# adaly/gridnext

Hardware: AMD Instinct MI355X
Metric: spots/sec training throughput (multimodal f+g) (higher is better)
Workload: dtype f32; 1 GPU; C4: multimodal f(DenseNet-121 @128px + count-MLP 2000 genes) + hex g on 78x64 Visium grids, 1 array (4992 spots) per GPU per step, f frozen/eval (tutorial mode), g trained with Adam, masked CE; spots_per_array=4992, parallelism=dp1

## Files before the change

### gridnext_amd/_lib.py

```python
import ctypes
import os

import torch

_HERE = os.path.dirname(os.path.abspath(__file__))
LIB_PATH = os.environ.get('GNX_LIB') or os.path.join(_HERE, 'libgridnext_hip.so')

_P, _I, _L, _F, _D = ctypes.c_void_p, ctypes.c_int, ctypes.c_long, ctypes.c_float, ctypes.c_double
_LL = ctypes.c_longlong

SIGNATURES = {
    'gnx_hexconv_fwd': (_I, [_P, _P, _P, _P, _P, _I, _I, _I, _I, _I, _I, _P]),
    'gnx_hexconv_bwd_data': (_I, [_P, _P, _P, _P, _I, _I, _I, _I, _I, _I, _P]),
    'gnx_hexconv_bwd_weight_workspace': (_L, [_I, _I, _I, _I, _I]),
    'gnx_hexconv_bwd_weight': (_I, [_P, _P, _P, _P, _P, _P, _I, _I, _I, _I, _I, _I, _I, _P]),
    'gnx_hexconv_bwd_weight_batch': (_I, [_P, _I, _P]),
    'gnx_hexconv_k_fwd': (_I, [_P, _P, _P, _P, _I, _I, _I, _I, _I, _I, _I, _P]),
    'gnx_hexconv_k_bwd_data': (_I, [_P, _P, _P, _I, _I, _I, _I, _I, _I, _I, _P]),
    'gnx_hexconv_k_bwd_weight_workspace': (_L, [_I, _I, _I, _I, _I, _I]),
    'gnx_hexconv_k_bwd_weight': (_I, [_P, _P, _P, _P, _P, _I, _I, _I, _I, _I, _I, _I, _I, _P]),
    'gnx_gridconv_fwd': (_I, [_P, _P, _P, _P, _I, _I, _I, _I, _I, _I, _I, _P]),
    'gnx_gridconv_bwd_data': (_I, [_P, _P, _P, _I, _I, _I, _I, _I, _I, _I, _P]),
    'gnx_gridconv_bwd_weight_workspace': (_L, [_I, _I, _I, _I, _I, _I, _I]),
    'gnx_gridconv_bwd_weight': (_I, [_P, _P, _P, _P, _P, _I, _I, _I, _I, _I, _I, _I, _I, _P]),
# ... 79 lines not shown
    'gnx_trans_bwd_f16': (_I, [_P, _L, _P, _L, _P, _L, _L, _I, _I, _P, _P, _P, _P, _P, _P, _P, _P, _I, _P, _P]),
    'gnx_h16_cols_to_f32': (_I, [_P, _L, _P, _L, _L, _I, _P, _P, _P]),
    'gnx_stem_bwd_f16_workspace': (_L, [_L, _I]),
    'gnx_stem_bwd_f16': (_I, [_P, _P, _P, _P, _P, _P, _P, _L, _P, _P, _P, _P, _L, _I, _I, _P, _I, _P, _P]),
    'gnx_dense_layer_f16_pack': (_I, [_P, _P, _P, _P, _I, _P]),
    'gnx_dense_layer_f16': (_I, [_P, _L, _L, _I, _I, _P, _P, _P, _P, _P, _P, _P]),
    'gnx_dense_layer_f16_tape': (_I, [_P, _L, _L, _I, _I, _P, _P, _P, _P, _P, _P, _P, _L, _P]),
    'gnx_dense_bwd_f16_pack': (_I, [_P, _P, _P, _P, _I, _P]),
    'gnx_wgrad3x3_f16_lb': (_I, [_P, _L, _P, _L, _L, _P, _P, _L, _I, _P, _I, _P, _P]),
    'gnx_conv3x3_dgrad_bnrelu_bwd_f16_lb': (_I, [_P, _L, _P, _P, _L, _L, _P, _L, _I, _P, _P, _P, _P, _P, _P, _P, _I, _P, _P]),
    'gnx_conv3x3_bwd_f16_workspace': (_L, [_L]),
    'gnx_conv3x3_bwd_f16_lb': (_I, [_P, _L, _P, _P, _L, _L, _P, _P, _L, _I, _P, _P, _P, _P, _P, _P, _P, _I, _P, _P]),
    'gnx_conv1x1_dgrad_wgrad_bnrelu_bwd_f16_lb': (_I, [_P, _P, _P, _L, _L, _P, _L, _L, _L, _I, _P, _P, _P, _P, _P, _P, _P, _P, _P, _I,
                                                       _P, _P]),
    'gnx_tail_bwd_f16_lb': (_I, [_P, _L, _P, _L, _L, _P, _L, _L, _L, _I, _I, _P, _P, _P, _P, _P, _P, _P, _P, _I, _P, _P]),
    'gnx_trans_bwd_f16_lb': (_I, [_P, _L, _L, _P, _L, _L, _P, _L, _L, _L, _I, _I, _P, _P, _P, _P, _P, _P, _P, _P, _I, _P, _P]),
    'gnx_conv_stem_bnrelu_maxpool_f16mul_cb': (_I, [_P, _I, _P, _P, _L, _L, _I, _I, _I, _I, _I, _I, _I, _I, _P, _P, _P, _P]),
    'gnx_conv1x1_bnrelu_h16_cb': (_I, [_P, _L, _P, _P, _L, _L, _I, _I, _P, _P, _P, _P, _P]),
    'gnx_bnrelu_avgpool2_h16_cb': (_I, [_P, _L, _P, _L, _L, _I, _I, _P, _P, _P]),
    'gnx_transition_f16_pack': (_I, [_P, _P, _I, _I, _P]),
    'gnx_transition_f16': (_I, [_P, _L, _L, _I, _I, _I, _P, _P, _P, _P, _L, _P]),
    'gnx_transition_f16_tape': (_I, [_P, _L, _L, _I, _I, _I, _P, _P, _P, _P, _L, _P, _L, _P]),
    'gnx_bnrelu_avgpool_h16_cb': (_I, [_P, _L, _P, _L, _L, _I, _I, _P, _P, _P]),
    'gnx_conv3x3_bnrelu': (_I, [_P, _L, _P, _P, _L, _L, _I, _I, _I, _P, _P, _P]),
    'gnx_winograd_conv3x3_weights': (_I, [_P, _P, _I, _I, _P]),
    'gnx_conv3x3_winograd': (_I, [_P, _L, _P, _P, _L, _L, _I, _I, _I, _P]),
    'gnx_conv3x3_winograd_wide': (_I, [_P, _L, _P, _P, _L, _L, _I, _I, _I, _P]),
    'gnx_conv3x3_form': (_I, [_P, _L, _P, _P, _L, _L, _I, _I, _I, _P, _P, _P]),
    'gnx_conv3x3_winograd_form': (_I, [_P, _L, _P, _P, _L, _L, _I, _I, _I, _P]),
    'gnx_conv3x3_dgrad_bnrelu_bwd_form': (_I, [_P, _L, _P, _P, _L, _P, _L, _L, _I, _I, _I, _P, _P, _P, _P, _P, _P]),
    'gnx_conv3x3_f16_dma_form': (_I, [_P, _L, _P, _P, _L, _L, _I, _I, _I, _P]),
    'gnx_conv_stem': (_I, [_P, _P, _P, _L, _L, _I, _I, _I, _I, _I, _I, _I, _I, _P]),
    'gnx_conv_stem_bnrelu_maxpool': (_I, [_P, _P, _P, _L, _L, _I, _I, _I, _I, _I, _I, _I, _I, _P, _P, _P]),
    'gnx_conv_stem_bnrelu_maxpool_argmax': (_I, [_P, _P, _P, _L, _P, _L, _I, _I, _I, _I, _I, _I, _I, _I, _P, _P, _P]),
    'gnx_bnrelu_maxpool': (_I, [_P, _L, _P, _L, _L, _I, _I, _I, _P, _P, _P]),
    'gnx_bnrelu_avgpool': (_I, [_P, _L, _P, _L, _L, _I, _I, _P, _P, _P]),
    'gnx_spot_compact': (_I, [_P, _L, _L, _P, _P, _P, _P, _P]),
    'gnx_spot_broadcast_rows': (_I, [_P, _L, _L, _I, _P, _L, _P]),
    'gnx_conv_stem_bnrelu_maxpool_idx': (_I, [_P, _P, _P, _L, _L, _I, _I, _I, _I, _I, _I, _I, _I, _P, _P, _P, _L, _P]),
    'gnx_conv_stem_bnrelu_maxpool_u8_idx': (_I, [_P, _P, _P, _L, _L, _I, _I, _I, _I, _I, _I, _I, _I, _P, _P, _P, _P, _L, _P]),
    'gnx_bnrelu_avgpool_idx': (_I, [_P, _L, _P, _L, _L, _I, _I, _P, _P, _P, _L, _P]),
    'gnx_wgrad_workspace': (_L, [_L, _I, _I, _I]),
    'gnx_wgrad_bnrelu': (_I, [_P, _L, _P, _L, _P, _P, _P, _P, _L, _I, _I, _I, _I, _I, _I, _P]),
    'gnx_wgrad_bnrelu_batch': (_I, [_P, _I, _I, _P]),
    'gnx_transpose_weight': (_I, [_P, _P, _I, _I, _P]),
    'gnx_relayout_weights_batch': (_I, [_P, _I, _I, _P]),
    'gnx_repack_conv3x3_bwd': (_I, [_P, _P, _I, _I, _P]),
    'gnx_rows_broadcast': (_I, [_P, _L, _P, _L, _L, _I, _I, _F, _P]),
    'gnx_avgpool2_bwd': (_I, [_P, _L, _P, _L, _L, _I, _I, _P]),
    'gnx_maxpool_bwd': (_I, [_P, _L, _P, _L, _P, _L, _P, _L, _L, _I, _I, _I, _P, _P, _P]),
    'gnx_bnrelu_maxpool_argmax': (_I, [_P, _L, _P, _L, _P, _L, _I, _I, _I, _P, _P, _P]),
    'gnx_maxpool_bwd_argmax': (_I, [_P, _P, _L, _P, _L, _L, _I, _I, _I, _P]),
    'gnx_maxpool_bwd_argmax_bnrelu': (_I, [_P, _P, _L, _P, _L, _P, _P, _L, _L, _I, _I, _I, _P]),
    'gnx_conv0_wgrad_workspace': (_L, [_L, _I, _I, _I, _I, _I, _I, _I]),
    'gnx_conv0_wgrad': (_I, [_P, _P, _L, _P, _P, _L, _I, _I, _I, _I, _I, _I, _I, _I, _P]),
    'gnx_conv0_dgrad': (_I, [_P, _L, _P, _P, _L, _I, _I, _I, _I, _I, _I, _I, _P]),
    'gnx_softmax_rows': (_I, [_P, _L, _L, _I, _P, _L, _P, _P]),
    'gnx_gemm_f32': (_I, [_P, _L, _I, _P, _L, _I, _P, _P, _L, _L, _L, _L, _I, _P]),
    'gnx_gemm_f32_workspace': (_L, [_L, _L, _L]),
    'gnx_gemm_f32_ws': (_I, [_P, _L, _I, _P, _L, _I, _P, _P, _L, _L, _L, _L, _I, _P, _P]),
    'gnx_fingerprint128_split_bytes': (_L, []),
    'gnx_fingerprint128_batch_workspace': (_L, [ctypes.c_size_t, _I]),
    'gnx_fingerprint128_batch': (_I, [_P, ctypes.c_size_t, _I, _P, _P, _P]),
    'gnx_rgb_hist_u8_workspace': (_L, [ctypes.c_size_t]),
    'gnx_rgb_hist_u8': (_I, [_P, ctypes.c_size_t, _P, _P, _P]),
    'gnx_rgb_lut_u8': (_I, [_P, _P, ctypes.c_size_t, _P, _P]),
# ... 69 lines not shown
```

### gridnext_amd/csrc/stem_pool.hip

```cpp
#include <type_traits>
#include "fwd_common.h"

namespace {

__global__ __launch_bounds__(256) void u8_to_f32_kernel(const uint8_t* __restrict__ x8, float* __restrict__ out, long n4,
                                                        long hw4, int C, const float* __restrict__ nrm) {
    const long stride = (long)gridDim.x * blockDim.x;
    for (long i = (long)blockIdx.x * blockDim.x + threadIdx.x; i < n4; i += stride) {
        const int c = (int)((i / hw4) % C);
        const bool norm = nrm != nullptr && c < 3;
        const float mean = norm ? nrm[c] : 0.f, sd = norm ? nrm[3 + c] : 1.f, rsd = norm ? nrm[6 + c] : 1.f;
        const uint32_t wv = reinterpret_cast<const uint32_t*>(x8)[i];
        reinterpret_cast<float4*>(out)[i] = u8x4_pixels(wv, norm, mean, sd, rsd);
    }
}

constexpr int ST_BM = 128, ST_BN = 64;

__global__ __launch_bounds__(256) void conv_stem_kernel(const float* __restrict__ x, const float* __restrict__ w,
                                                        float* __restrict__ out, long ldc, long M, int Cin, int H,
                                                        int Wd, int Ho, int Wo, int O, int KH, int KW, int stride,
                                                        int pad) {
    extern __shared__ __attribute__((aligned(16))) float lds[];
    const int KC = KH * 8, LD = KC + 4;
// ... 131 lines not shown
            float4 na = a, nb0 = b0, nb1 = b1;
            if (step + 1 < NSTEP) {
                na = load_a(step + 1);
                nb0 = ld4(pb + (step + 1) * 8);
                nb1 = ld4(pb + 32 * LDB + (step + 1) * 8);
            }
            acc0 = __builtin_amdgcn_mfma_f32_32x32x2f32(a.x, b0.x, acc0, 0, 0, 0);
            acc1 = __builtin_amdgcn_mfma_f32_32x32x2f32(a.x, b1.x, acc1, 0, 0, 0);
            acc0 = __builtin_amdgcn_mfma_f32_32x32x2f32(a.y, b0.y, acc0, 0, 0, 0);
            acc1 = __builtin_amdgcn_mfma_f32_32x32x2f32(a.y, b1.y, acc1, 0, 0, 0);
            acc0 = __builtin_amdgcn_mfma_f32_32x32x2f32(a.z, b0.z, acc0, 0, 0, 0);
            acc1 = __builtin_amdgcn_mfma_f32_32x32x2f32(a.z, b1.z, acc1, 0, 0, 0);
            acc0 = __builtin_amdgcn_mfma_f32_32x32x2f32(a.w, b0.w, acc0, 0, 0, 0);
            acc1 = __builtin_amdgcn_mfma_f32_32x32x2f32(a.w, b1.w, acc1, 0, 0, 0);
            a = na; b0 = nb0; b1 = nb1;
            __builtin_amdgcn_sched_group_barrier(0x100, STRIDE % 2 == 0 ? 4 : 6, 0);
            __builtin_amdgcn_sched_group_barrier(0x008, 8, 0);
        }
#pragma unroll
        for (int r = 0; r < 16; ++r) {
            const int rr = 32 * wave + (r & 3) + 8 * (r >> 2) + 4 * h;
            const int oy = oy0 + (rr >> 4), ox = ox0 + (rr & 15);
            if (oy < Ho && ox < Wo) {
                float* o = out + ((img * Ho + oy) * (long)Wo + ox) * ldc;
                if (i < O) o[i] = acc0[r];
                if (32 + i < O) o[32 + i] = acc1[r];
            }
        }
    }
}

constexpr int SP_LDT = 40;
constexpr int SP_LDTH = 72;
template <int WO, bool H16 = false, bool U8 = false, bool IDX = false>
__global__ __launch_bounds__(256) void conv_stem_pool_kernel(const void* __restrict__ xv, const float* __restrict__ w,
                                                             float* __restrict__ out, long ldo, int H, int Wd, int O,
                                                             const float* __restrict__ scale,
                                                             const float* __restrict__ shift, long imgs,
                                                             const float* __restrict__ nrm,
                                                             unsigned char* __restrict__ amax = nullptr,
                                                             const int* __restrict__ src_idx = nullptr, long src_imgs = 0) {
    const float* __restrict__ x = reinterpret_cast<const float*>(xv);
    const uint8_t* __restrict__ x8 = reinterpret_cast<const uint8_t*>(xv);
    constexpr int CIN = 3, KH = 7, KW = 7, STRIDE = 2, PAD = 3;
    constexpr int RT = 128 / WO;
    constexpr int PH = STRIDE * (RT - 1) + KH, PW = ((WO - 1) * STRIDE + 8 + 1 + 1) & ~1;
    constexpr int F4R = WO * STRIDE / 4;
    constexpr int NPC = CIN * PH * F4R, NPRE = (NPC + 255) / 256;
    constexpr int NIT = (WO / 2) * 8 / 256;
    constexpr int KT = CIN * KH * 8, LDB = KT + 4;
    extern __shared__ __attribute__((aligned(16))) float lds[];
    auto store4 = [](float* o, long off, const float4& v) {
        if constexpr (H16) {
            typedef _Float16 half4 __attribute__((ext_vector_type(4)));
            const half4 hv = {(_Float16)v.x, (_Float16)v.y, (_Float16)v.z, (_Float16)v.w};
            *reinterpret_cast<half4*>(reinterpret_cast<_Float16*>(o) + off) = hv;
        } else {
            *reinterpret_cast<float4*>(o + off) = v;
        }
    };
    float* Bs = lds;
    float* Ps = lds + 64 * LDB;
    float* Ts = Ps + CIN * PH * PW;
    const int t = threadIdx.x, lane = t & 63, wave = t >> 6, h = lane >> 5, i = lane & 31;
    for (int idx = t; idx < 64 * KT; idx += 256) {
        const int n = idx / KT, rem = idx - n * KT;
        const int kx = rem & 7, cky = rem >> 3;
        float v = 0.f;
        if (n < O && kx < KW) v = w[((long)n * CIN * KH + cky) * KW + kx];
        Bs[n * LDB + rem] = v;
    }
    for (int idx = t; idx < CIN * PH * PW; idx += 256) Ps[idx] = 0.f;
    const int trow = 32 * wave + i;
    const float* pa = Ps + (STRIDE * (trow / WO)) * PW + STRIDE * (trow % WO) + 4 * h;
    const float* pb = Bs + i * LDB + 4 * h;
    const float sc0 = i < O ? scale[i] : 0.f, sh0 = i < O ? shift[i] : 0.f;
    const float sc1 = 32 + i < O ? scale[32 + i] : 0.f, sh1 = 32 + i < O ? shift[32 + i] : 0.f;
    const int c4 = t & 7, pxa = t >> 3;
    const int Ho2 = (H + 2 * PAD - KH) / STRIDE + 1;
    const int ntt = Ho2 / RT;

    float4 pre[U8 ? 1 : NPRE];
    uint32_t pre8[U8 ? NPRE : 1];
    bool in8[U8 ? NPRE : 1];
    auto fetch_patch = [&](long img, int tt) {
        const int iy0 = RT * tt * STRIDE - PAD;
#pragma unroll
        for (int q = 0; q < NPRE; ++q) {
            const int j = t + 256 * q;
            const int f4 = j % F4R, py = (j / F4R) % PH, c = (j / F4R) / PH;
            const int iy = iy0 + py;
            const bool inside = j < NPC && iy >= 0 && iy < H;
            if constexpr (U8) {
                pre8[q] = 0u;
                in8[q] = inside;
                if (inside)
                    pre8[q] = *reinterpret_cast<const uint32_t*>(x8 + ((img * CIN + c) * H + iy) * (long)Wd + 4 * f4);
            } else {
                pre[q] = make_float4(0.f, 0.f, 0.f, 0.f);
                if (inside) pre[q] = ld4(x + ((img * CIN + c) * H + iy) * (long)Wd + 4 * f4);
            }
        }
    };
    auto stash_patch = [&]() {
#pragma unroll
        for (int q = 0; q < NPRE; ++q) {
            const int j = t + 256 * q;
            if (j < NPC) {
                float* d = Ps + (j / F4R) * PW + PAD + 4 * (j % F4R);
                if constexpr (U8) {
                    const int c = (j / F4R) / PH;
                    const bool norm = nrm != nullptr;
                    const float4 v = in8[q] ? u8x4_pixels(pre8[q], norm, norm ? nrm[c] : 0.f, norm ? nrm[3 + c] : 1.f,
                                                          norm ? nrm[6 + c] : 1.f)
                                            : make_float4(0.f, 0.f, 0.f, 0.f);
                    d[0] = v.x; d[1] = v.y; d[2] = v.z; d[3] = v.w;
                } else {
                    d[0] = pre[q].x; d[1] = pre[q].y; d[2] = pre[q].z; d[3] = pre[q].w;
                }
            }
        }
    };
    auto src_of = [&](long img) -> long {
        if (src_idx == nullptr) return img;
        const long s = src_idx[img];
        return s < 0 ? 0 : (s < src_imgs ? s : src_imgs - 1);
    };
    __syncthreads();
    fetch_patch(src_of(blockIdx.x), 0);

    for (long img = blockIdx.x; img < imgs; img += gridDim.x) {
        const long src = src_of(img);
        float4 carry[2][NIT], carry2[2][NIT];
        unsigned cidx[2][NIT], cidx2[2][NIT];
        const float c0v = IDX ? -1.f : 0.f;
#pragma unroll
        for (int q = 0; q < NIT; ++q) {
            carry[0][q] = carry[1][q] = carry2[0][q] = carry2[1][q] = make_float4(c0v, c0v, c0v, c0v);
            cidx[0][q] = cidx[1][q] = cidx2[0][q] = cidx2[1][q] = 0u;
        }
        for (int tt = 0; tt < ntt; ++tt) {
            __syncthreads();
            stash_patch();
            {
                long nsrc = src;
                int nt2 = tt + 1;
                if (nt2 == ntt) {
                    nt2 = 0;
                    long nimg = img + gridDim.x;
                    if (nimg >= imgs) nimg = blockIdx.x;
                    nsrc = src_of(nimg);
                }
                fetch_patch(nsrc, nt2);
            }
            asm volatile("" ::: "memory");
            __syncthreads();
            f32x16 acc0, acc1;
#pragma unroll
            for (int r = 0; r < 16; ++r) { acc0[r] = 0.f; acc1[r] = 0.f; }
            auto load_a = [&](int step) {
                const float* ap = pa + ((step / KH) * PH + (step % KH)) * PW;
                const float2 lo = *reinterpret_cast<const float2*>(ap);
                const float2 hi = *reinterpret_cast<const float2*>(ap + 2);
                return make_float4(lo.x, lo.y, hi.x, hi.y);
            };
            constexpr int NSTEP = CIN * KH;
            float4 a = load_a(0), b0 = ld4(pb), b1 = ld4(pb + 32 * LDB);
#pragma unroll
            for (int step = 0; step < NSTEP; ++step) {
                float4 na = a, nb0 = b0, nb1 = b1;
                if (step + 1 < NSTEP) {
                    na = load_a(step + 1);
                    nb0 = ld4(pb + (step + 1) * 8);
                    nb1 = ld4(pb + 32 * LDB + (step + 1) * 8);
                }
                acc0 = __builtin_amdgcn_mfma_f32_32x32x2f32(a.x, b0.x, acc0, 0, 0, 0);
                acc1 = __builtin_amdgcn_mfma_f32_32x32x2f32(a.x, b1.x, acc1, 0, 0, 0);
                acc0 = __builtin_amdgcn_mfma_f32_32x32x2f32(a.y, b0.y, acc0, 0, 0, 0);
                acc1 = __builtin_amdgcn_mfma_f32_32x32x2f32(a.y, b1.y, acc1, 0, 0, 0);
                acc0 = __builtin_amdgcn_mfma_f32_32x32x2f32(a.z, b0.z, acc0, 0, 0, 0);
                acc1 = __builtin_amdgcn_mfma_f32_32x32x2f32(a.z, b1.z, acc1, 0, 0, 0);
                acc0 = __builtin_amdgcn_mfma_f32_32x32x2f32(a.w, b0.w, acc0, 0, 0, 0);
                acc1 = __builtin_amdgcn_mfma_f32_32x32x2f32(a.w, b1.w, acc1, 0, 0, 0);
                a = na; b0 = nb0; b1 = nb1;
                __builtin_amdgcn_sched_group_barrier(0x100, 4, 0);
                __builtin_amdgcn_sched_group_barrier(0x008, 8, 0);
            }
#pragma unroll
            for (int pass = 0; pass < 2; ++pass) {
                if (pass == 1) __syncthreads();
#pragma unroll
                for (int r = 0; r < 16; ++r) {
                    const int rr = 32 * wave + (r & 3) + 8 * (r >> 2) + 4 * h;
                    Ts[rr * SP_LDT + i] = pass == 0 ? fmaxf(fmaf(acc0[r], sc0, sh0), 0.f) : fmaxf(fmaf(acc1[r], sc1, sh1), 0.f);
                }
                __syncthreads();
                const int ch = 32 * pass + 4 * c4;
#pragma unroll
                for (int q = 0; q < NIT; ++q) {
                    const int px = pxa + 32 * q;
                    float4 m0 = make_float4(c0v, c0v, c0v, c0v), m1 = m0;
                    unsigned h0 = 0u, h1 = 0u;
                    auto hmax = [](float4& m, unsigned& hx, const float4& v, unsigned col) {
                        if (IDX) {
                            if (v.x > m.x) { m.x = v.x; hx = (hx & 0xffffff00u) | col; }
                            if (v.y > m.y) { m.y = v.y; hx = (hx & 0xffff00ffu) | (col << 8); }
                            if (v.z > m.z) { m.z = v.z; hx = (hx & 0xff00ffffu) | (col << 16); }
                            if (v.w > m.w) { m.w = v.w; hx = (hx & 0x00ffffffu) | (col << 24); }
                        } else {
                            m = make_float4(fmaxf(m.x, v.x), fmaxf(m.y, v.y), fmaxf(m.z, v.z), fmaxf(m.w, v.w));
                        }
                    };
#pragma unroll
                    for (int dx = -1; dx <= 1; ++dx) {
                        const int ox = 2 * px + dx;
                        if (ox < 0) continue;
                        hmax(m0, h0, ld4(&Ts[ox * SP_LDT + 4 * c4]), (unsigned)(dx + 1));
                        if (RT == 2) hmax(m1, h1, ld4(&Ts[(WO + ox) * SP_LDT + 4 * c4]), (unsigned)(dx + 1));
                    }
                    auto vmax = [](const float4& ra, unsigned ia, const float4& rb, unsigned ib, const float4& rc, unsigned ic,
                                   float4& o4, unsigned& oi) {
                        if (IDX) {
                            o4 = ra; oi = ia;
                            const unsigned jb = ib + 0x03030303u, jc = ic + 0x06060606u;
                            if (rb.x > o4.x) { o4.x = rb.x; oi = (oi & 0xffffff00u) | (jb & 0x000000ffu); }
                            if (rb.y > o4.y) { o4.y = rb.y; oi = (oi & 0xffff00ffu) | (jb & 0x0000ff00u); }
                            if (rb.z > o4.z) { o4.z = rb.z; oi = (oi & 0xff00ffffu) | (jb & 0x00ff0000u); }
                            if (rb.w > o4.w) { o4.w = rb.w; oi = (oi & 0x00ffffffu) | (jb & 0xff000000u); }
                            if (rc.x > o4.x) { o4.x = rc.x; oi = (oi & 0xffffff00u) | (jc & 0x000000ffu); }
// ... 335 lines not shown
}

}

GNX_EXPORT int gnx_conv_stem(const float* x, const float* w, float* out, long ldc, long imgs, int Cin, int H, int W,
                             int O, int KH, int KW, int stride, int pad, hipStream_t stream) {
    if (!x || !w || !out || imgs < 0 || Cin <= 0 || O <= 0 || KH <= 0 || KH > 7 || KW <= 0 || KW > 8 || stride <= 0 ||
        ldc < O)
        return GNX_ERR_BAD_ARG;
    const int Ho = (H + 2 * pad - KH) / stride + 1, Wo = (W + 2 * pad - KW) / stride + 1;
    if (Ho <= 0 || Wo <= 0) return GNX_ERR_BAD_ARG;
    const long M = imgs * Ho * Wo;
    if (M == 0) return GNX_OK;
    if (O <= 64 && Cin == 3 && ((stride == 2 && KH == 7 && KW == 7) || (stride == 1 && KH == 3 && KW == 3))) {
        const int tiles_x = gnx_cdiv(Wo, 16), tiles_y = gnx_cdiv(Ho, 8);
        const long ntiles = imgs * tiles_x * tiles_y;
        const int PH = 7 * stride + KH, PW = (15 * stride + 8 + 1) & ~1;
        const size_t lds2 = ((size_t)64 * (Cin * KH * 8 + 4) + (size_t)Cin * PH * PW) * sizeof(float);
        const int grid2 = (int)(ntiles < 256 * 3 ? ntiles : 256 * 3);
        if (stride == 2)
            conv_stem_patch_kernel<2, 7, 3><<<grid2, 256, lds2, stream>>>(x, w, out, ldc, Cin, H, W, Ho, Wo, O, KW, pad,
                                                                      tiles_x, tiles_y, ntiles);
        else
            conv_stem_patch_kernel<1, 3, 3><<<grid2, 256, lds2, stream>>>(x, w, out, ldc, Cin, H, W, Ho, Wo, O, KW, pad,
                                                                      tiles_x, tiles_y, ntiles);
        return gnx_launch_status();
    }
    const size_t lds_bytes = (size_t)(ST_BM + ST_BN) * (KH * 8 + 4) * sizeof(float);
    dim3 grid(gnx_cdiv(M, ST_BM), gnx_cdiv(O, ST_BN));
    conv_stem_kernel<<<grid, 256, lds_bytes, stream>>>(x, w, out, ldc, M, Cin, H, W, Ho, Wo, O, KH, KW, stride, pad);
    return gnx_launch_status();
}

template <bool H16, bool U8 = false>
static int stem_pool_launch(const void* x, const float* w, float* out, long ldo, long imgs, int Cin, int H, int W, int O,
                            int KH, int KW, int stride, int pad, const float* scale, const float* shift, hipStream_t stream,
                            const float* nrm = nullptr, unsigned char* amax = nullptr, const int* src_idx = nullptr,
                            long src_imgs = 0) {
    if (!x || !w || !out || !scale || !shift || imgs < 0 || Cin <= 0 || O <= 0 || H <= 0 || W <= 0 || ldo < O)
        return GNX_ERR_BAD_ARG;
    if (src_idx && (src_imgs <= 0 || amax)) return GNX_ERR_BAD_ARG;
    if (amax && (H16 || U8 || (reinterpret_cast<uintptr_t>(amax) & 3) != 0)) return GNX_ERR_UNSUPPORTED;
    if (Cin != 3 || KH != 7 || KW != 7 || stride != 2 || pad != 3 || O > 64 || O % 4 != 0 || ldo % 4 != 0 ||
        (reinterpret_cast<uintptr_t>(out) & (H16 ? 7 : 15)) != 0)
        return GNX_ERR_UNSUPPORTED;
    const int Ho = (H + 6 - 7) / 2 + 1, Wo = (W + 6 - 7) / 2 + 1;
    if ((Wo != 64 && Wo != 128) || W != 2 * Wo || Ho % 2 != 0 || Ho <= 0 ||
        (reinterpret_cast<uintptr_t>(x) & (U8 ? 3 : 15)) != 0)
        return GNX_ERR_UNSUPPORTED;
    if (imgs == 0) return GNX_OK;
    const int RT = 128 / Wo, PH = 2 * (RT - 1) + 7, PW = ((Wo - 1) * 2 + 8 + 2) & ~1;
    const size_t lds_bytes = ((size_t)64 * (3 * 7 * 8 + 4) + (size_t)3 * PH * PW + (size_t)128 * SP_LDT) * sizeof(float);
    const int per_cu = lds_bytes <= 80 * 1024 ? 2 : 1;
    const int grid = (int)(imgs < 256 * per_cu ? imgs : 256 * per_cu);
    if (Wo == 64) {
        static bool conf = false;
        if (!conf) {
            if (hipFuncSetAttribute(reinterpret_cast<const void*>(conv_stem_pool_kernel<64, H16, U8>),
                                    hipFuncAttributeMaxDynamicSharedMemorySize, (int)lds_bytes) != hipSuccess)
                return GNX_ERR_LAUNCH;
            conf = true;
        }
        if constexpr (!H16 && !U8) {
            if (amax) {
                static bool confi = false;
                if (!confi) {
                    if (hipFuncSetAttribute(reinterpret_cast<const void*>(conv_stem_pool_kernel<64, false, false, true>),
                                            hipFuncAttributeMaxDynamicSharedMemorySize, (int)lds_bytes) != hipSuccess)
                        return GNX_ERR_LAUNCH;
                    confi = true;
                }
                conv_stem_pool_kernel<64, false, false, true><<<grid, 256, lds_bytes, stream>>>(x, w, out, ldo, H, W, O, scale,
                                                                                                shift, imgs, nrm, amax);
                return gnx_launch_status();
            }
        }
        conv_stem_pool_kernel<64, H16, U8><<<grid, 256, lds_bytes, stream>>>(x, w, out, ldo, H, W, O, scale, shift, imgs, nrm,
                                                                             nullptr, src_idx, src_imgs);
    } else {
        static bool conf = false;
        if (!conf) {
            if (hipFuncSetAttribute(reinterpret_cast<const void*>(conv_stem_pool_kernel<128, H16, U8>),
                                    hipFuncAttributeMaxDynamicSharedMemorySize, (int)lds_bytes) != hipSuccess)
                return GNX_ERR_LAUNCH;
            conf = true;
        }
        if constexpr (!H16 && !U8) {
            if (amax) {
                static bool confi = false;
                if (!confi) {
                    if (hipFuncSetAttribute(reinterpret_cast<const void*>(conv_stem_pool_kernel<128, false, false, true>),
                                            hipFuncAttributeMaxDynamicSharedMemorySize, (int)lds_bytes) != hipSuccess)
                        return GNX_ERR_LAUNCH;
                    confi = true;
                }
                conv_stem_pool_kernel<128, false, false, true><<<grid, 256, lds_bytes, stream>>>(x, w, out, ldo, H, W, O, scale,
                                                                                                 shift, imgs, nrm, amax);
                return gnx_launch_status();
            }
        }
        conv_stem_pool_kernel<128, H16, U8><<<grid, 256, lds_bytes, stream>>>(x, w, out, ldo, H, W, O, scale, shift, imgs, nrm,
                                                                              nullptr, src_idx, src_imgs);
    }
    return gnx_launch_status();
}
GNX_EXPORT int gnx_conv_stem_bnrelu_maxpool(const float* x, const float* w, float* out, long ldo, long imgs, int Cin,
                                            int H, int W, int O, int KH, int KW, int stride, int pad, const float* scale,
                                            const float* shift, hipStream_t stream) {
    return stem_pool_launch<false>(x, w, out, ldo, imgs, Cin, H, W, O, KH, KW, stride, pad, scale, shift, stream);
}
GNX_EXPORT int gnx_conv_stem_bnrelu_maxpool_idx(const float* x, const float* w, float* out, long ldo, long imgs, int Cin,
                                                int H, int W, int O, int KH, int KW, int stride, int pad, const float* scale,
                                                const float* shift, const int* src_idx, long src_imgs, hipStream_t stream) {
    if (!src_idx) return GNX_ERR_BAD_ARG;
    return stem_pool_launch<false>(x, w, out, ldo, imgs, Cin, H, W, O, KH, KW, stride, pad, scale, shift, stream, nullptr,
                                   nullptr, src_idx, src_imgs);
}
GNX_EXPORT int gnx_conv_stem_bnrelu_maxpool_argmax(const float* x, const float* w, float* out, long ldo,
                                                   unsigned char* argmax, long imgs, int Cin, int H, int W, int O, int KH,
                                                   int KW, int stride, int pad, const float* scale, const float* shift,
                                                   hipStream_t stream) {
    if (!argmax) return GNX_ERR_BAD_ARG;
    return stem_pool_launch<false>(x, w, out, ldo, imgs, Cin, H, W, O, KH, KW, stride, pad, scale, shift, stream, nullptr,
                                   argmax);
}
GNX_EXPORT int gnx_conv_stem_bnrelu_maxpool_h16(const float* x, const float* w, void* out16, long ldo, long imgs, int Cin,
                                                int H, int W, int O, int KH, int KW, int stride, int pad,
                                                const float* scale, const float* shift, hipStream_t stream) {
    return stem_pool_launch<true>(x, w, reinterpret_cast<float*>(out16), ldo, imgs, Cin, H, W, O, KH, KW, stride, pad, scale,
                                  shift, stream);
}

template <bool U8>
static int stem_pool_f16_launch(const void* x, const float* w, void* out16, long ldo, long imgs, int Cin, int H, int W, int O,
                                int KH, int KW, int stride, int pad, const float* scale, const float* shift,
                                const float* nrm, hipStream_t stream, long obs = 32) {
    if (!x || !w || !out16 || !scale || !shift || imgs < 0 || Cin <= 0 || O <= 0 || H <= 0 || W <= 0 ||
        (obs == 32 ? ldo < O : ldo != 32))
        return GNX_ERR_BAD_ARG;
    if (Cin != 3 || KH != 7 || KW != 7 || stride != 2 || pad != 3 || O > 64 || O % 4 != 0 || ldo % 4 != 0 ||
        (reinterpret_cast<uintptr_t>(out16) & 7) != 0)
        return GNX_ERR_UNSUPPORTED;
// ... 153 lines not shown
```

### include/gridnext_hip.h

```cpp
#ifndef GRIDNEXT_HIP_H
#define GRIDNEXT_HIP_H

#include <stddef.h>
#include <stdint.h>

#ifdef __cplusplus
extern "C" {
#endif

#define GNX_OK 0
#define GNX_ERR_BAD_ARG (-1)
#define GNX_ERR_LAUNCH (-2)
#define GNX_ERR_UNSUPPORTED (-3)

typedef void* gnx_stream_t;

int gnx_hexconv_fwd(const float* x, const float* kernel0, const float* kernel1, const float* bias, float* y,
                    int B, int H, int W, int I, int O, int mode, gnx_stream_t stream);
int gnx_hexconv_bwd_data(const float* dy, const float* kernel0, const float* kernel1, float* dx,
                         int B, int H, int W, int I, int O, int mode, gnx_stream_t stream);
long gnx_hexconv_bwd_weight_workspace(int B, int H, int W, int I, int O);
int gnx_hexconv_bwd_weight(const float* x, const float* dy, float* dkernel0, float* dkernel1, float* dbias,
                           float* workspace, int B, int H, int W, int I, int O, int mode, int accumulate,
                           gnx_stream_t stream);
// ... 147 lines not shown
int gnx_repack_conv3x3(const float* w, float* wr, int N, int K, gnx_stream_t stream);
int gnx_conv3x3_bnrelu(const float* A, long lda, const float* Wr, float* out, long ldc, long M, int N, int K, int S,
                       const float* scale, const float* shift, gnx_stream_t stream);
int gnx_winograd_conv3x3_weights(const float* w, float* wu, int N, int K, gnx_stream_t stream);
int gnx_conv3x3_winograd(const float* A, long lda, const float* Wu, float* out, long ldc, long M, int N, int K, int S,
                         gnx_stream_t stream);
int gnx_conv3x3_winograd_wide(const float* A, long lda, const float* Wu, float* out, long ldc, long M, int N, int K, int S,
                              gnx_stream_t stream);
#define GNX_C3_GENERIC 0
#define GNX_C3_PIPE5 1
#define GNX_C3_PIPE6 2
#define GNX_C3_PIPE7 3
#define GNX_C3_PIPE9 4
#define GNX_C3_DMA4 5
#define GNX_C3_DMA8 6
#define GNX_C3_DMAG4 7
#define GNX_C3_DMAG8 8
#define GNX_C3_WINO 9
#define GNX_C3_WINO8 10
int gnx_conv3x3_form(const float* A, long lda, const float* Wr, const float* out, long ldc, long M, int N, int K, int S,
                     const float* scale, const float* shift, int* workgroups);
int gnx_conv3x3_winograd_form(const float* A, long lda, const float* Wu, const float* out, long ldc, long M, int N, int K, int S,
                              int* workgroups);
int gnx_conv3x3_dgrad_bnrelu_bwd_form(const float* dY, long lddy, const float* Wb, const float* A_act, long lda, const float* dX,
                                      long lddx, long M, int N, int K, int S, const float* scale, const float* shift,
                                      const float* mean, const float* invstd, const float* workspace, int* workgroups);
int gnx_conv3x3_f16_dma_form(const void* A16, long lda16, const void* Wr16, const void* out, long ldc, long M, int N, int K,
                             int S, int* workgroups);
int gnx_conv_stem(const float* x, const float* w, float* out, long ldc, long imgs, int Cin, int H, int W, int O,
                  int KH, int KW, int stride, int pad, gnx_stream_t stream);
int gnx_conv_stem_bnrelu_maxpool(const float* x, const float* w, float* out, long ldo, long imgs, int Cin, int H, int W,
                                 int O, int KH, int KW, int stride, int pad, const float* scale, const float* shift,
                                 gnx_stream_t stream);
int gnx_conv_stem_bnrelu_maxpool_argmax(const float* x, const float* w, float* out, long ldo, unsigned char* argmax,
                                        long imgs, int Cin, int H, int W, int O, int KH, int KW, int stride, int pad,
                                        const float* scale, const float* shift, gnx_stream_t stream);
int gnx_bnrelu_maxpool(const float* in, long ldi, float* out, long ldo, long imgs, int C, int Hi, int Wi,
                       const float* scale, const float* shift, gnx_stream_t stream);
int gnx_bnrelu_avgpool(const float* in, long ldi, float* out, long ldo, long imgs, int C, int S2,
                       const float* scale, const float* shift, gnx_stream_t stream);

int gnx_spot_compact(const void* x, long spot_bytes, long N, int* flags, int* fg_idx, int* bg_idx, int* counts,
                     gnx_stream_t stream);
int gnx_spot_broadcast_rows(float* rows, long ld, long n_rows, int C, const int* bg_idx, long n_bg, gnx_stream_t stream);
int gnx_conv_stem_bnrelu_maxpool_idx(const float* x, const float* w, float* out, long ldo, long imgs, int Cin, int H, int W,
                                     int O, int KH, int KW, int stride, int pad, const float* scale, const float* shift,
                                     const int* src_idx, long src_imgs, gnx_stream_t stream);
int gnx_conv_stem_bnrelu_maxpool_u8_idx(const unsigned char* x8, const float* w, float* out, long ldo, long imgs, int Cin,
                                        int H, int W, int O, int KH, int KW, int stride, int pad, const float* scale,
                                        const float* shift, const float* norm, const int* src_idx, long src_imgs,
                                        gnx_stream_t stream);
int gnx_bnrelu_avgpool_idx(const float* in, long ldi, float* out, long ldo, long imgs, int C, int S2, const float* scale,
                           const float* shift, const int* dst_idx, long dst_rows, gnx_stream_t stream);

int gnx_conv1x1_bnrelu_f16(const float* A, long lda, const float* W, float* out, long ldc, long M, int N, int K,
                           const float* scale, const float* shift, int pool, int S_in, gnx_stream_t stream);
int gnx_conv3x3_bnrelu_f16(const float* A, long lda, const float* Wr, float* out, long ldc, long M, int N, int K, int S,
                           const float* scale, const float* shift, gnx_stream_t stream);
int gnx_conv1x1_bnrelu_f16_act16(const float* A, long lda, const float* W, void* out16, long ldc16, long M, int N, int K,
                                 const float* scale, const float* shift, const float* out_scale, const float* out_shift,
                                 gnx_stream_t stream);
int gnx_conv3x3_f16_dma(const void* A16, long lda16, const void* Wr16, float* out, long ldc, long M, int N, int K, int S,
                        gnx_stream_t stream);
int gnx_conv_stem_bnrelu_maxpool_h16(const float* x, const float* w, void* out16, long ldo, long imgs, int Cin, int H, int W,
                                     int O, int KH, int KW, int stride, int pad, const float* scale, const float* shift,
                                     gnx_stream_t stream);
// ... 183 lines not shown
```

Before: 87650 spots/s.

## Pack stem conv K dimension densely, reuse overlapping patch rows, use buffer loads

The default stem conv+BN+ReLU+maxpool kernel now packs the 7-wide kernel taps densely into K, dropping the pad-to-8 zero columns, so fewer MFMA steps run per tile. It also keeps the overlapping input rows between consecutive row tiles in LDS and fetches only the new rows, instead of restaging the full patch each tile. Global patch fetches switch to raw buffer loads with out-of-range offsets returning zero, and the old pad-8 path stays available as a separate export. In exchange the indexing gets more complex, extra LDS move and sync steps are added per tile, and the Wo=128 case is forced to one block per CU.

```diff
diff --git a/gridnext_amd/_lib.py b/gridnext_amd/_lib.py
--- a/gridnext_amd/_lib.py
+++ b/gridnext_amd/_lib.py
@@ -135,6 +135,7 @@
     'gnx_conv3x3_f16_dma_form': (_I, [_P, _L, _P, _P, _L, _L, _I, _I, _I, _P]),
     'gnx_conv_stem': (_I, [_P, _P, _P, _L, _L, _I, _I, _I, _I, _I, _I, _I, _I, _P]),
     'gnx_conv_stem_bnrelu_maxpool': (_I, [_P, _P, _P, _L, _L, _I, _I, _I, _I, _I, _I, _I, _I, _P, _P, _P]),
+    'gnx_conv_stem_bnrelu_maxpool_pad8': (_I, [_P, _P, _P, _L, _L, _I, _I, _I, _I, _I, _I, _I, _I, _P, _P, _P]),
     'gnx_conv_stem_bnrelu_maxpool_argmax': (_I, [_P, _P, _P, _L, _P, _L, _I, _I, _I, _I, _I, _I, _I, _I, _P, _P, _P]),
     'gnx_bnrelu_maxpool': (_I, [_P, _L, _P, _L, _L, _I, _I, _I, _P, _P, _P]),
     'gnx_bnrelu_avgpool': (_I, [_P, _L, _P, _L, _L, _I, _I, _P, _P, _P]),
diff --git a/gridnext_amd/csrc/stem_pool.hip b/gridnext_amd/csrc/stem_pool.hip
--- a/gridnext_amd/csrc/stem_pool.hip
+++ b/gridnext_amd/csrc/stem_pool.hip
@@ -187,7 +187,19 @@
 
 constexpr int SP_LDT = 40;
 constexpr int SP_LDTH = 72;
-template <int WO, bool H16 = false, bool U8 = false, bool IDX = false>
+#ifndef GNX_STEM_PAD8
+#define GNX_STEM_PAD8 0
+#endif
+#ifndef GNX_STEM_FLAT
+#define GNX_STEM_FLAT 0
+#endif
+#ifndef GNX_STEM_FULLSTAGE
+#define GNX_STEM_FULLSTAGE 0
+#endif
+constexpr int SP_LDW = 76;
+constexpr int SP_LDB = 3 * 7 * 8 + 4;
+constexpr int sp_weight_floats(bool pad8) { return pad8 ? 64 * SP_LDB : 128 * SP_LDW; }
+template <int WO, bool H16 = false, bool U8 = false, bool IDX = false, bool PAD8 = (GNX_STEM_PAD8 != 0)>
 __global__ __launch_bounds__(256) void conv_stem_pool_kernel(const void* __restrict__ xv, const float* __restrict__ w,
                                                              float* __restrict__ out, long ldo, int H, int Wd, int O,
                                                              const float* __restrict__ scale,
@@ -201,9 +213,15 @@
     constexpr int RT = 128 / WO;
     constexpr int PH = STRIDE * (RT - 1) + KH, PW = ((WO - 1) * STRIDE + 8 + 1 + 1) & ~1;
     constexpr int F4R = WO * STRIDE / 4;
-    constexpr int NPC = CIN * PH * F4R, NPRE = (NPC + 255) / 256;
+    constexpr bool SHIFT = GNX_STEM_FULLSTAGE == 0;
+    constexpr int NEWR = SHIFT ? RT * STRIDE : PH, KEEP = PH - NEWR, TT0 = SHIFT ? -1 : 0;
+    constexpr int NPC = CIN * NEWR * F4R, NPRE = (NPC + 255) / 256;
+    constexpr int PW4 = PW / 4, NMV = CIN * KEEP * PW4, NMVT = (NMV + 255) / 256;
+    constexpr int KP4 = KEEP > 0 ? KEEP * PW4 : 1, ZP4 = KEEP > NEWR ? (KEEP - NEWR) * PW4 : 1;
+    static_assert(PW % 4 == 0 && (CIN * PH * PW) % 4 == 0, "16-B rows");
     constexpr int NIT = (WO / 2) * 8 / 256;
-    constexpr int KT = CIN * KH * 8, LDB = KT + 4;
+    constexpr int KT = CIN * KH * 8, LDB = SP_LDB, LDW = SP_LDW;
+    constexpr int NG = CIN * KH;
     extern __shared__ __attribute__((aligned(16))) float lds[];
     auto store4 = [](float* o, long off, const float4& v) {
         if constexpr (H16) {
@@ -215,20 +233,45 @@
         }
     };
     float* Bs = lds;
-    float* Ps = lds + 64 * LDB;
+    float* Ps = lds + sp_weight_floats(PAD8);
     float* Ts = Ps + CIN * PH * PW;
     const int t = threadIdx.x, lane = t & 63, wave = t >> 6, h = lane >> 5, i = lane & 31;
-    for (int idx = t; idx < 64 * KT; idx += 256) {
-        const int n = idx / KT, rem = idx - n * KT;
-        const int kx = rem & 7, cky = rem >> 3;
-        float v = 0.f;
-        if (n < O && kx < KW) v = w[((long)n * CIN * KH + cky) * KW + kx];
-        Bs[n * LDB + rem] = v;
+    if constexpr (PAD8) {
+        for (int idx = t; idx < 64 * KT; idx += 256) {
+            const int n = idx / KT, rem = idx - n * KT;
+            const int kx = rem & 7, cky = rem >> 3;
+            float v = 0.f;
+            if (n < O && kx < KW) v = w[((long)n * CIN * KH + cky) * KW + kx];
+            Bs[n * LDB + rem] = v;
+        }
+    } else {
+        for (int idx = t; idx < 128 * LDW; idx += 256) {
+            const int hh = idx / (64 * LDW), r = idx - hh * 64 * LDW, n = r / LDW, p = r - n * LDW;
+            int g = NG - 1, kx = p - 70 + 4 * hh;
+            if (p < 70) {
+                const int m = p / 7, q = p - 7 * m;
+                const bool first = q < 4 - hh;
+                g = 2 * m + (first ? 0 : 1);
+                kx = hh ? (first ? q + 4 : q - 3) : q;
+            }
+            float v = 0.f;
+            if (n < O && p < 74 && kx < KW) v = w[((long)n * NG + g) * KW + kx];
+            Bs[idx] = v;
+        }
     }
     for (int idx = t; idx < CIN * PH * PW; idx += 256) Ps[idx] = 0.f;
     const int trow = 32 * wave + i;
-    const float* pa = Ps + (STRIDE * (trow / WO)) * PW + STRIDE * (trow % WO) + 4 * h;
-    const float* pb = Bs + i * LDB + 4 * h;
+    const float* pa0 = Ps + (STRIDE * (trow / WO)) * PW + STRIDE * (trow % WO);
+    const float* pa = pa0 + 4 * h;
+    const float* pc = pa0 + 4 - 3 * h;
+    int one = 1, two = 2;
+    asm volatile("" : "+v"(one), "+v"(two));
+    const float* pc5 = pc + one;
+    const float* pc6 = pc + two;
+    constexpr int DCH = (PH - (KH - 1)) * PW;
+    const float* p3 = pa0 + (h ? PW : 3);
+    const float* p3c = pa0 + (h ? DCH : 3);
+    const float* pb = PAD8 ? Bs + i * LDB + 4 * h : Bs + (64 * h + i) * LDW;
     const float sc0 = i < O ? scale[i] : 0.f, sh0 = i < O ? shift[i] : 0.f;
     const float sc1 = 32 + i < O ? scale[32 + i] : 0.f, sh1 = 32 + i < O ? shift[32 + i] : 0.f;
     const int c4 = t & 7, pxa = t >> 3;
@@ -239,21 +282,34 @@
     uint32_t pre8[U8 ? NPRE : 1];
     bool in8[U8 ? NPRE : 1];
     auto fetch_patch = [&](long img, int tt) {
-        const int iy0 = RT * tt * STRIDE - PAD;
+        const int iy0 = RT * tt * STRIDE - PAD + KEEP;
+        const unsigned esz = U8 ? 1u : 4u, ibytes = (unsigned)(CIN * H * Wd) * esz;
+        const __amdgpu_buffer_rsrc_t rx = __builtin_amdgcn_make_buffer_rsrc(
+            const_cast<uint8_t*>(x8) + img * (long)ibytes, 0, ibytes, 0x00020000);
 #pragma unroll
         for (int q = 0; q < NPRE; ++q) {
             const int j = t + 256 * q;
-            const int f4 = j % F4R, py = (j / F4R) % PH, c = (j / F4R) / PH;
+            const int f4 = j % F4R, py = (j / F4R) % NEWR, c = (j / F4R) / NEWR;
             const int iy = iy0 + py;
             const bool inside = j < NPC && iy >= 0 && iy < H;
-            if constexpr (U8) {
-                pre8[q] = 0u;
-                in8[q] = inside;
-                if (inside)
-                    pre8[q] = *reinterpret_cast<const uint32_t*>(x8 + ((img * CIN + c) * H + iy) * (long)Wd + 4 * f4);
+            if constexpr (GNX_STEM_FLAT != 0) {
+                if constexpr (U8) {
+                    pre8[q] = 0u;
+                    in8[q] = inside;
+                    if (inside)
+                        pre8[q] = *reinterpret_cast<const uint32_t*>(x8 + ((img * CIN + c) * H + iy) * (long)Wd + 4 * f4);
+                } else {
+                    pre[q] = make_float4(0.f, 0.f, 0.f, 0.f);
+                    if (inside) pre[q] = ld4(x + ((img * CIN + c) * H + iy) * (long)Wd + 4 * f4);
+                }
             } else {
-                pre[q] = make_float4(0.f, 0.f, 0.f, 0.f);
-                if (inside) pre[q] = ld4(x + ((img * CIN + c) * H + iy) * (long)Wd + 4 * f4);
+                const unsigned voff = inside ? (unsigned)((c * H + iy) * Wd + 4 * f4) * esz : 0x80000000u;
+                if constexpr (U8) {
+                    in8[q] = inside;
+                    pre8[q] = __builtin_amdgcn_raw_buffer_load_b32(rx, voff, 0, 0);
+                } else {
+                    pre[q] = __builtin_bit_cast(float4, __builtin_amdgcn_raw_buffer_load_b128(rx, voff, 0, 0));
+                }
             }
         }
     };
@@ -262,9 +318,9 @@
         for (int q = 0; q < NPRE; ++q) {
             const int j = t + 256 * q;
             if (j < NPC) {
-                float* d = Ps + (j / F4R) * PW + PAD + 4 * (j % F4R);
+                const int c = (j / F4R) / NEWR, py = KEEP + (j / F4R) % NEWR;
+                float* d = Ps + (c * PH + py) * PW + PAD + 4 * (j % F4R);
                 if constexpr (U8) {
-                    const int c = (j / F4R) / PH;
                     const bool norm = nrm != nullptr;
                     const float4 v = in8[q] ? u8x4_pixels(pre8[q], norm, norm ? nrm[c] : 0.f, norm ? nrm[3 + c] : 1.f,
                                                           norm ? nrm[6 + c] : 1.f)
@@ -281,8 +337,23 @@
         const long s = src_idx[img];
         return s < 0 ? 0 : (s < src_imgs ? s : src_imgs - 1);
     };
+    float4 mv[NMVT > 0 ? NMVT : 1];
+    auto move_read = [&]() {
+#pragma unroll
+        for (int q = 0; q < NMVT; ++q) {
+            const int j = t + 256 * q, c = j / KP4, r = j - c * KP4;
+            if (j < NMV) mv[q] = ld4(Ps + (c * PH + NEWR) * PW + 4 * r);
+        }
+    };
+    auto move_write = [&]() {
+#pragma unroll
+        for (int q = 0; q < NMVT; ++q) {
+            const int j = t + 256 * q, c = j / KP4, r = j - c * KP4;
+            if (j < NMV) *reinterpret_cast<float4*>(Ps + c * PH * PW + 4 * r) = mv[q];
+        }
+    };
     __syncthreads();
-    fetch_patch(src_of(blockIdx.x), 0);
+    fetch_patch(src_of(blockIdx.x), TT0);
 
     for (long img = blockIdx.x; img < imgs; img += gridDim.x) {
         const long src = src_of(img);
@@ -294,14 +365,20 @@
             carry[0][q] = carry[1][q] = carry2[0][q] = carry2[1][q] = make_float4(c0v, c0v, c0v, c0v);
             cidx[0][q] = cidx[1][q] = cidx2[0][q] = cidx2[1][q] = 0u;
         }
-        for (int tt = 0; tt < ntt; ++tt) {
+        for (int tt = TT0; tt < ntt; ++tt) {
             __syncthreads();
             stash_patch();
+            if (SHIFT && tt < 0) {
+                for (int j = t; j < CIN * ZP4; j += 256) {
+                    const int c = j / ZP4, r = j - c * ZP4;
+                    *reinterpret_cast<float4*>(Ps + (c * PH + NEWR) * PW + 4 * r) = make_float4(0.f, 0.f, 0.f, 0.f);
+                }
+            }
             {
                 long nsrc = src;
                 int nt2 = tt + 1;
                 if (nt2 == ntt) {
-                    nt2 = 0;
+                    nt2 = TT0;
                     long nimg = img + gridDim.x;
                     if (nimg >= imgs) nimg = blockIdx.x;
                     nsrc = src_of(nimg);
@@ -310,37 +387,89 @@
             }
             asm volatile("" ::: "memory");
             __syncthreads();
+            if (SHIFT && tt < 0) {
+                move_read();
+                __syncthreads();
+                move_write();
+                continue;
+            }
             f32x16 acc0, acc1;
 #pragma unroll
             for (int r = 0; r < 16; ++r) { acc0[r] = 0.f; acc1[r] = 0.f; }
-            auto load_a = [&](int step) {
-                const float* ap = pa + ((step / KH) * PH + (step % KH)) * PW;
-                const float2 lo = *reinterpret_cast<const float2*>(ap);
-                const float2 hi = *reinterpret_cast<const float2*>(ap + 2);
-                return make_float4(lo.x, lo.y, hi.x, hi.y);
-            };
-            constexpr int NSTEP = CIN * KH;
-            float4 a = load_a(0), b0 = ld4(pb), b1 = ld4(pb + 32 * LDB);
-#pragma unroll
-            for (int step = 0; step < NSTEP; ++step) {
-                float4 na = a, nb0 = b0, nb1 = b1;
-                if (step + 1 < NSTEP) {
-                    na = load_a(step + 1);
-                    nb0 = ld4(pb + (step + 1) * 8);
-                    nb1 = ld4(pb + 32 * LDB + (step + 1) * 8);
-                }
-                acc0 = __builtin_amdgcn_mfma_f32_32x32x2f32(a.x, b0.x, acc0, 0, 0, 0);
-                acc1 = __builtin_amdgcn_mfma_f32_32x32x2f32(a.x, b1.x, acc1, 0, 0, 0);
-                acc0 = __builtin_amdgcn_mfma_f32_32x32x2f32(a.y, b0.y, acc0, 0, 0, 0);
-                acc1 = __builtin_amdgcn_mfma_f32_32x32x2f32(a.y, b1.y, acc1, 0, 0, 0);
-                acc0 = __builtin_amdgcn_mfma_f32_32x32x2f32(a.z, b0.z, acc0, 0, 0, 0);
-                acc1 = __builtin_amdgcn_mfma_f32_32x32x2f32(a.z, b1.z, acc1, 0, 0, 0);
-                acc0 = __builtin_amdgcn_mfma_f32_32x32x2f32(a.w, b0.w, acc0, 0, 0, 0);
-                acc1 = __builtin_amdgcn_mfma_f32_32x32x2f32(a.w, b1.w, acc1, 0, 0, 0);
-                a = na; b0 = nb0; b1 = nb1;
-                __builtin_amdgcn_sched_group_barrier(0x100, 4, 0);
-                __builtin_amdgcn_sched_group_barrier(0x008, 8, 0);
-            }
+            if constexpr (PAD8) {
+                auto load_a = [&](int step) {
+                    const float* ap = pa + ((step / KH) * PH + (step % KH)) * PW;
+                    const float2 lo = *reinterpret_cast<const float2*>(ap);
+                    const float2 hi = *reinterpret_cast<const float2*>(ap + 2);
+                    return make_float4(lo.x, lo.y, hi.x, hi.y);
+                };
+                constexpr int NSTEP = CIN * KH;
+                float4 a = load_a(0), b0 = ld4(pb), b1 = ld4(pb + 32 * LDB);
+    #pragma unroll
+                for (int step = 0; step < NSTEP; ++step) {
+                    float4 na = a, nb0 = b0, nb1 = b1;
+                    if (step + 1 < NSTEP) {
+                        na = load_a(step + 1);
+                        nb0 = ld4(pb + (step + 1) * 8);
+                        nb1 = ld4(pb + 32 * LDB + (step + 1) * 8);
+                    }
+                    acc0 = __builtin_amdgcn_mfma_f32_32x32x2f32(a.x, b0.x, acc0, 0, 0, 0);
+                    acc1 = __builtin_amdgcn_mfma_f32_32x32x2f32(a.x, b1.x, acc1, 0, 0, 0);
+                    acc0 = __builtin_amdgcn_mfma_f32_32x32x2f32(a.y, b0.y, acc0, 0, 0, 0);
+                    acc1 = __builtin_amdgcn_mfma_f32_32x32x2f32(a.y, b1.y, acc1, 0, 0, 0);
+                    acc0 = __builtin_amdgcn_mfma_f32_32x32x2f32(a.z, b0.z, acc0, 0, 0, 0);
+                    acc1 = __builtin_amdgcn_mfma_f32_32x32x2f32(a.z, b1.z, acc1, 0, 0, 0);
+                    acc0 = __builtin_amdgcn_mfma_f32_32x32x2f32(a.w, b0.w, acc0, 0, 0, 0);
+                    acc1 = __builtin_amdgcn_mfma_f32_32x32x2f32(a.w, b1.w, acc1, 0, 0, 0);
+                    a = na; b0 = nb0; b1 = nb1;
+                    __builtin_amdgcn_sched_group_barrier(0x100, 4, 0);
+                    __builtin_amdgcn_sched_group_barrier(0x008, 8, 0);
+                }
+            } else {
+                auto rowoff = [](int g) { return ((g / KH) * PH + (g % KH)) * PW; };
+                auto load_a = [&](int m, float (&r)[7]) {
+                    const int o0 = rowoff(2 * m);
+                    const float2 v01 = *reinterpret_cast<const float2*>(pa + o0);
+                    r[0] = v01.x; r[1] = v01.y;
+                    if (m == NG / 2) {
+                        const float2 v23 = *reinterpret_cast<const float2*>(pa + o0 + 2);
+                        r[2] = v23.x; r[3] = v23.y;
+                        return;
+                    }
+                    const int o1 = rowoff(2 * m + 1);
+                    r[2] = pa[o0 + 2];
+                    r[3] = (o1 - o0 == PW ? p3 : p3c)[o0];
+                    r[4] = pc[o1]; r[5] = pc5[o1]; r[6] = pc6[o1];
+                };
+                float a[7], na[7];
+                float4 b0 = ld4(pb), b1 = ld4(pb + 32 * LDW), nb0 = b0, nb1 = b1;
+                load_a(0, a);
+                static_for<0, NG / 2 + 1>([&](auto mc) {
+                    constexpr int m = decltype(mc)::value, np = m < NG / 2 ? 7 : 4;
+                    if constexpr (m < NG / 2) load_a(m + 1, na);
+                    constexpr int p0 = 7 * m, v0 = (p0 + 3) / 4 + 1, v1 = (p0 + np - 1) / 4 + 1;
+                    constexpr int nbv = (v1 < LDW / 4 ? v1 : LDW / 4 - 1) - v0 + 1;
+#pragma unroll
+                    for (int q = 0; q < np; ++q) {
+                        const int p = p0 + q, e = p & 3;
+                        if (e == 0 && p + 4 < LDW) {
+                            nb0 = ld4(pb + p + 4);
+                            nb1 = ld4(pb + 32 * LDW + p + 4);
+                        }
+                        const float w0 = e == 0 ? b0.x : e == 1 ? b0.y : e == 2 ? b0.z : b0.w;
+                        const float w1 = e == 0 ? b1.x : e == 1 ? b1.y : e == 2 ? b1.z : b1.w;
+                        acc0 = __builtin_amdgcn_mfma_f32_32x32x2f32(a[q], w0, acc0, 0, 0, 0);
+                        acc1 = __builtin_amdgcn_mfma_f32_32x32x2f32(a[q], w1, acc1, 0, 0, 0);
+                        if (e == 3) { b0 = nb0; b1 = nb1; }
+                    }
+#pragma unroll
+                    for (int q = 0; q < 7; ++q) a[q] = na[q];
+                    constexpr int nrd = (m + 1 < NG / 2 ? 6 : m < NG / 2 ? 2 : 0) + 2 * (nbv > 0 ? nbv : 0);
+                    __builtin_amdgcn_sched_group_barrier(0x100, nrd, 0);
+                    __builtin_amdgcn_sched_group_barrier(0x008, 2 * np, 0);
+                });
+            }
+            if constexpr (SHIFT) move_read();
 #pragma unroll
             for (int pass = 0; pass < 2; ++pass) {
                 if (pass == 1) __syncthreads();
@@ -350,6 +479,7 @@
                     Ts[rr * SP_LDT + i] = pass == 0 ? fmaxf(fmaf(acc0[r], sc0, sh0), 0.f) : fmaxf(fmaf(acc1[r], sc1, sh1), 0.f);
                 }
                 __syncthreads();
+                if (SHIFT && pass == 0) move_write();
                 const int ch = 32 * pass + 4 * c4;
 #pragma unroll
                 for (int q = 0; q < NIT; ++q) {
@@ -751,7 +881,7 @@
     return gnx_launch_status();
 }
 
-template <bool H16, bool U8 = false>
+template <bool H16, bool U8 = false, bool P8 = (GNX_STEM_PAD8 != 0)>
 static int stem_pool_launch(const void* x, const float* w, float* out, long ldo, long imgs, int Cin, int H, int W, int O,
                             int KH, int KW, int stride, int pad, const float* scale, const float* shift, hipStream_t stream,
                             const float* nrm = nullptr, unsigned char* amax = nullptr, const int* src_idx = nullptr,
@@ -769,13 +899,13 @@
         return GNX_ERR_UNSUPPORTED;
     if (imgs == 0) return GNX_OK;
     const int RT = 128 / Wo, PH = 2 * (RT - 1) + 7, PW = ((Wo - 1) * 2 + 8 + 2) & ~1;
-    const size_t lds_bytes = ((size_t)64 * (3 * 7 * 8 + 4) + (size_t)3 * PH * PW + (size_t)128 * SP_LDT) * sizeof(float);
-    const int per_cu = lds_bytes <= 80 * 1024 ? 2 : 1;
+    const size_t lds_bytes = ((size_t)sp_weight_floats(P8) + (size_t)3 * PH * PW + (size_t)128 * SP_LDT) * sizeof(float);
+    const int per_cu = Wo == 64 ? 2 : 1;
     const int grid = (int)(imgs < 256 * per_cu ? imgs : 256 * per_cu);
     if (Wo == 64) {
         static bool conf = false;
         if (!conf) {
-            if (hipFuncSetAttribute(reinterpret_cast<const void*>(conv_stem_pool_kernel<64, H16, U8>),
+            if (hipFuncSetAttribute(reinterpret_cast<const void*>(conv_stem_pool_kernel<64, H16, U8, false, P8>),
                                     hipFuncAttributeMaxDynamicSharedMemorySize, (int)lds_bytes) != hipSuccess)
                 return GNX_ERR_LAUNCH;
             conf = true;
@@ -784,22 +914,22 @@
             if (amax) {
                 static bool confi = false;
                 if (!confi) {
-                    if (hipFuncSetAttribute(reinterpret_cast<const void*>(conv_stem_pool_kernel<64, false, false, true>),
+                    if (hipFuncSetAttribute(reinterpret_cast<const void*>(conv_stem_pool_kernel<64, false, false, true, P8>),
                                             hipFuncAttributeMaxDynamicSharedMemorySize, (int)lds_bytes) != hipSuccess)
                         return GNX_ERR_LAUNCH;
                     confi = true;
                 }
-                conv_stem_pool_kernel<64, false, false, true><<<grid, 256, lds_bytes, stream>>>(x, w, out, ldo, H, W, O, scale,
+                conv_stem_pool_kernel<64, false, false, true, P8><<<grid, 256, lds_bytes, stream>>>(x, w, out, ldo, H, W, O, scale,
                                                                                                 shift, imgs, nrm, amax);
                 return gnx_launch_status();
             }
         }
-        conv_stem_pool_kernel<64, H16, U8><<<grid, 256, lds_bytes, stream>>>(x, w, out, ldo, H, W, O, scale, shift, imgs, nrm,
+        conv_stem_pool_kernel<64, H16, U8, false, P8><<<grid, 256, lds_bytes, stream>>>(x, w, out, ldo, H, W, O, scale, shift, imgs, nrm,
                                                                              nullptr, src_idx, src_imgs);
     } else {
         static bool conf = false;
         if (!conf) {
-            if (hipFuncSetAttribute(reinterpret_cast<const void*>(conv_stem_pool_kernel<128, H16, U8>),
+            if (hipFuncSetAttribute(reinterpret_cast<const void*>(conv_stem_pool_kernel<128, H16, U8, false, P8>),
                                     hipFuncAttributeMaxDynamicSharedMemorySize, (int)lds_bytes) != hipSuccess)
                 return GNX_ERR_LAUNCH;
             conf = true;
@@ -808,17 +938,17 @@
             if (amax) {
                 static bool confi = false;
                 if (!confi) {
-                    if (hipFuncSetAttribute(reinterpret_cast<const void*>(conv_stem_pool_kernel<128, false, false, true>),
+                    if (hipFuncSetAttribute(reinterpret_cast<const void*>(conv_stem_pool_kernel<128, false, false, true, P8>),
                                             hipFuncAttributeMaxDynamicSharedMemorySize, (int)lds_bytes) != hipSuccess)
                         return GNX_ERR_LAUNCH;
                     confi = true;
                 }
-                conv_stem_pool_kernel<128, false, false, true><<<grid, 256, lds_bytes, stream>>>(x, w, out, ldo, H, W, O, scale,
+                conv_stem_pool_kernel<128, false, false, true, P8><<<grid, 256, lds_bytes, stream>>>(x, w, out, ldo, H, W, O, scale,
                                                                                                  shift, imgs, nrm, amax);
                 return gnx_launch_status();
             }
         }
-        conv_stem_pool_kernel<128, H16, U8><<<grid, 256, lds_bytes, stream>>>(x, w, out, ldo, H, W, O, scale, shift, imgs, nrm,
+        conv_stem_pool_kernel<128, H16, U8, false, P8><<<grid, 256, lds_bytes, stream>>>(x, w, out, ldo, H, W, O, scale, shift, imgs, nrm,
                                                                               nullptr, src_idx, src_imgs);
     }
     return gnx_launch_status();
@@ -827,6 +957,12 @@
                                             int H, int W, int O, int KH, int KW, int stride, int pad, const float* scale,
                                             const float* shift, hipStream_t stream) {
     return stem_pool_launch<false>(x, w, out, ldo, imgs, Cin, H, W, O, KH, KW, stride, pad, scale, shift, stream);
+}
+GNX_EXPORT int gnx_conv_stem_bnrelu_maxpool_pad8(const float* x, const float* w, float* out, long ldo, long imgs, int Cin,
+                                                 int H, int W, int O, int KH, int KW, int stride, int pad, const float* scale,
+                                                 const float* shift, hipStream_t stream) {
+    if (W != 128) return GNX_ERR_UNSUPPORTED;
+    return stem_pool_launch<false, false, true>(x, w, out, ldo, imgs, Cin, H, W, O, KH, KW, stride, pad, scale, shift, stream);
 }
 GNX_EXPORT int gnx_conv_stem_bnrelu_maxpool_idx(const float* x, const float* w, float* out, long ldo, long imgs, int Cin,
                                                 int H, int W, int O, int KH, int KW, int stride, int pad, const float* scale,
diff --git a/include/gridnext_hip.h b/include/gridnext_hip.h
--- a/include/gridnext_hip.h
+++ b/include/gridnext_hip.h
@@ -203,6 +203,9 @@
 int gnx_conv_stem_bnrelu_maxpool(const float* x, const float* w, float* out, long ldo, long imgs, int Cin, int H, int W,
                                  int O, int KH, int KW, int stride, int pad, const float* scale, const float* shift,
                                  gnx_stream_t stream);
+int gnx_conv_stem_bnrelu_maxpool_pad8(const float* x, const float* w, float* out, long ldo, long imgs, int Cin, int H, int W,
+                                      int O, int KH, int KW, int stride, int pad, const float* scale, const float* shift,
+                                      gnx_stream_t stream);
 int gnx_conv_stem_bnrelu_maxpool_argmax(const float* x, const float* w, float* out, long ldo, unsigned char* argmax,
                                         long imgs, int Cin, int H, int W, int O, int KH, int KW, int stride, int pad,
                                         const float* scale, const float* shift, gnx_stream_t stream);
```

Measured after the change: 87030 spots/s (median of 2 runs). Within noise of the previous version (-0.7%).
